# vannem95/operational-space-control

Hardware: AMD Instinct MI355X
Metric: OSC control steps/sec (batched envs), Go2 18-DoF, at 1/2/4/8 MI355X (higher is better)
Workload: dtype f64; 1 GPU; unitree_go2 standing mask=ones, 4096 envs per GPU (BASELINE configs[1]); robot=unitree_go2, envs_per_gpu=4096, global_envs=4096, parallelism=env-shard x1

## Files before the change

### operational-space-control_amd/csrc/osc_setup.hpp

```cpp
#pragma once
#include "osc_device.hpp"
#include "osc_kin_device.hpp"
#include "osc_wave_sum.hpp"

namespace osc {

typedef double d4 __attribute__((ext_vector_type(4)));

__device__ __forceinline__ double wave_sum(double v) { return wave_sum_fast(v); }

template <int NR, int NDOT>
__device__ __forceinline__ void wave_mgs(double* rows, int stride, int ncol, int lane,
                                         double drop) {
  double a[NR];
  const bool cv = lane < ncol;
#pragma unroll
  for (int w = 0; w < NR; ++w) a[w] = cv ? rows[w * stride + lane] : 0.0;
  const bool dv = lane < NDOT;
#pragma unroll
  for (int w = 0; w < NR; ++w) {
    const double n0 = sqrt(wave_sum(dv ? a[w] * a[w] : 0.0));
#pragma unroll
    for (int v = 0; v < w; ++v) {
      const double cf = wave_sum(dv ? a[v] * a[w] : 0.0);
      a[w] = fma(-cf, a[v], a[w]);
    }
    const double nn = sqrt(wave_sum(dv ? a[w] * a[w] : 0.0));
    const double sc = (nn > drop * n0 && nn > 0.0) ? 1.0 / nn : 0.0;
    a[w] *= sc;
  }
  if (cv) {
#pragma unroll
    for (int w = 0; w < NR; ++w) rows[w * stride + lane] = a[w];
  }
}

template <int NROWS, int STRIDE, int NCOL, int NDOT>
__device__ __noinline__ void wave_mgs_lds(double* rows, int lane, double drop, double* scf) {
  const bool cv = lane < NCOL, dv = lane < NDOT;
  for (int w = 0; w < NROWS; ++w) {
    double aw = cv ? rows[w * STRIDE + lane] : 0.0;
    const double n0 = sqrt(wave_sum(dv ? aw * aw : 0.0));
    for (int pass = 0; pass < 2 && w > 0; ++pass) {
      double cf = 0.0;
      if (lane < w) {
        const double* rl = rows + lane * STRIDE;
        const double* rw = rows + w * STRIDE;
#pragma unroll
        for (int c = 0; c < NDOT; ++c) cf = fma(rl[c], rw[c], cf);
      }
      if (lane < w) scf[lane] = cf;
      __builtin_amdgcn_wave_barrier();
      asm volatile("" ::: "memory");
      if (cv) {
#pragma unroll 8
        for (int v = 0; v < w; ++v) aw = fma(-scf[v], rows[v * STRIDE + lane], aw);
        rows[w * STRIDE + lane] = aw;
      }
      __builtin_amdgcn_wave_barrier();
      asm volatile("" ::: "memory");
    }
    const double nn = sqrt(wave_sum(dv ? aw * aw : 0.0));
    const double sc = (nn > drop * n0 && nn > 0.0) ? 1.0 / nn : 0.0;
    if (cv) rows[w * STRIDE + lane] = aw * sc;
    __builtin_amdgcn_wave_barrier();
    asm volatile("" ::: "memory");
  }
}

template <class D, bool KIN = false, bool LEAN = false>
__device__ __forceinline__ void setup_env(
    const DevParams* __restrict__ P, int env, int nenv, const double* __restrict__ gM,
    const double* __restrict__ gC, const double* __restrict__ gJ, const double* __restrict__ gb,
    const double* __restrict__ gT, const double* __restrict__ gmask, double* __restrict__ ws,
    double* __restrict__ sm, const double* __restrict__ gwd,
    const osc_kin::KinDev* __restrict__ Kg = nullptr, const double* __restrict__ gqpos = nullptr,
    const double* __restrict__ gqvel = nullptr) {
  constexpr int NV = D::NV, NU = D::NU, NC = D::NC, NS = D::NS, NB = D::NB, NY = D::NY,
                NY1 = D::NY1, NY1P = D::NY1P, S = D::S, NA = D::NA;
  const int lane = threadIdx.x;
  if (env >= nenv) return;

  constexpr int NAP = D::NAP;
  double* sA = sm + D::O_A;
  double* sM = sm + D::O_M;
  double* sC = sm + D::O_C;
  constexpr bool kHaG = LEAN && !D::WH && !KIN;
  double* sHa = sm + (kHaG ? D::O_HD_L : D::O_HA);
  double* sX = sm + (kHaG ? D::O_X_L : D::O_X);
  double* sU = sX + NB * NY1P;
  double* sMask = sm + (kHaG ? D::O_MASK_L : D::O_MASK);

  STAMP_DECL
  STAMP_BEGIN();
  static_assert(NV % 2 == 0 && NC % 2 == 0, "16-byte staging needs even nv and nc");
  constexpr int JC0 = 3 * (NS - NC);
  constexpr int JR0 = D::JG ? JC0 : 0;
  constexpr int KSJ = D::JG ? (S + 3) / 4 : 0;
  double jf[KSJ > 0 ? KSJ : 1];
  Batch2<NC / 2, kWave> bK;
  bK.load(gmask + static_cast<size_t>(env) * NC, lane);
  if constexpr (!KIN) {
    Batch2<D::JROWS * NV / 2, kWave> bJ;
    Batch2<NV * NV / 2, kWave> bM;
    Batch2<NV / 2, kWave> bC;
    bJ.load(gJ + static_cast<size_t>(env) * S * NV + JR0 * NV, lane);
    bM.load(gM + static_cast<size_t>(env) * NV * NV, lane);
    bC.load(gC + static_cast<size_t>(env) * NV, lane);
    {
      const int lc = lane & 15, lg = lane >> 4;
#pragma unroll
      for (int q = 0; q < KSJ; ++q) {
        const int r = 4 * q + lg;
        jf[q] = gJ[static_cast<size_t>(env) * S * NV + (r < S ? r : S - 1) * NV + (lc < NV ? lc : 0)];
      }
    }
    constexpr int TEJ = D::JG ? (S + kWave - 1) / kWave : 0;
    double ebj[TEJ > 0 ? TEJ : 1], etj[TEJ > 0 ? TEJ : 1], wj[TEJ > 0 ? TEJ : 1];
#pragma unroll
    for (int q = 0; q < TEJ; ++q) {
      const int r = (lane + q * kWave < S) ? lane + q * kWave : S - 1;
      const int half = r / (3 * NS), rr = r % (3 * NS);
      ebj[q] = gb[static_cast<size_t>(env) * S + r];
      etj[q] = gT[static_cast<size_t>(env) * NS * 6 + (rr / 3) * 6 + half * 3 + rr % 3];
      wj[q] = P->w_row[r];
    }
    constexpr int TE = D::JG ? 0 : (S + kWave - 1) / kWave;
    double eb[TE > 0 ? TE : 1], et[TE > 0 ? TE : 1];
#pragma unroll
    for (int q = 0; q < TE; ++q) {
      const int r = (lane + q * kWave < S) ? lane + q * kWave : S - 1;
      const int half = r / (3 * NS), rr = r % (3 * NS);
      eb[q] = gb[static_cast<size_t>(env) * S + r];
      et[q] = gT[static_cast<size_t>(env) * NS * 6 + (rr / 3) * 6 + half * 3 + rr % 3];
    }
    bJ.store(sA, lane, [](int c) { return (c / (NV / 2)) * (NAP / 2) + c % (NV / 2); });
#pragma unroll
    for (int q = 0; q < TEJ; ++q) {
      const int r = (lane + q * kWave < S) ? lane + q * kWave : S - 1;
      sA[D::O_E + r] = ebj[q] - etj[q];
      sA[D::O_W + r] = wj[q];
    }
    bM.store(sM, lane);
    bC.store(sC, lane);
    bK.store(sMask, lane);
    if constexpr (D::WH) {
      double* wr = ws + static_cast<size_t>(env) * D::WS;
      bM.store(wr + D::W_RM, lane);
      bC.store(wr + D::W_RC, lane);
      bJ.store(wr + D::W_RJ, lane);
      static_assert(D::JG && D::JROWS == 3 * NC, "wheel rows: the contact rows are the staged ones");
      for (int q = lane; q < 3 * NC; q += kWave) wr[D::W_RB + q] = gb[static_cast<size_t>(env) * S + JC0 + q];
      for (int q = lane; q < 6 * NC; q += kWave) wr[D::W_RD + q] = gwd[static_cast<size_t>(env) * NC * 6 + q];
    }
#pragma unroll
    for (int q = 0; q < TE; ++q) {
      const int r = (lane + q * kWave < S) ? lane + q * kWave : S - 1;
      sA[r * NAP + NV] = eb[q] - et[q];
      if (NAP > NA) sA[r * NAP + NA] = 0.0;
    }
    wave_sync();
  } else {
    osc_kin::KinDev* sK = reinterpret_cast<osc_kin::KinDev*>(sm + D::O_HA);
    {
      static_assert(sizeof(osc_kin::KinDev) % 16 == 0 && D::O_HA % 2 == 0, "16-byte staging");
      const uint4* src = reinterpret_cast<const uint4*>(Kg);
      uint4* dst = reinterpret_cast<uint4*>(sK);
      for (int i = lane; i < static_cast<int>(sizeof(osc_kin::KinDev) / 16); i += kWave)
        dst[i] = src[i];
    }
    wave_sync();
    const osc_kin::KinDev* K = sK;
    const int nq = K->nq;
    const osc_kin::EnvLayout lay(nq, NV, K->nbody, NS);
    double* E = sm + D::O_HA + sizeof(osc_kin::KinDev) / 8;
    for (int i = lane; i < nq; i += kWave) E[lay.q + i] = gqpos[static_cast<size_t>(env) * nq + i];
    for (int i = lane; i < NV; i += kWave) E[lay.q + nq + i] = gqvel[static_cast<size_t>(env) * NV + i];
    wave_sync();
    osc_kin::kin_forward(K, E, lay, lane);
    osc_kin::kin_backward(K, E, lay, lane);
    for (int d = lane; d < NV; d += kWave) sC[d] = osc_kin::kin_dof(K, E, lay, d);
    double* wr = ws + static_cast<size_t>(env) * D::WS;
    for (int k = lane; k < NS; k += kWave) {
      double bp[3], br[3];
      osc_kin::kin_site(K, E, lay, k, bp, br);
      const double* Tk = gT + static_cast<size_t>(env) * NS * 6 + k * 6;
#pragma unroll
      for (int i = 0; i < 3; ++i) {
        const int rp = 3 * k + i, rr = 3 * NS + 3 * k + i;
        if constexpr (D::JG) {
          sA[D::O_E + rp] = bp[i] - Tk[i];
          sA[D::O_E + rr] = br[i] - Tk[3 + i];
        } else {
          sA[rp * NAP + NV] = bp[i] - Tk[i];
          sA[rr * NAP + NV] = br[i] - Tk[3 + i];
          if (NAP > NA) {
            sA[rp * NAP + NA] = 0.0;
            sA[rr * NAP + NA] = 0.0;
          }
        }
        if constexpr (D::WH) {
          if (k >= NS - NC) wr[D::W_RB + 3 * (k - (NS - NC)) + i] = bp[i];
        }
      }
    }
    if constexpr (D::JG) {
      for (int r = lane; r < S; r += kWave) sA[D::O_W + r] = P->w_row[r];
    }
    wave_sync();
    {
      const int j = lane & 31, par = lane >> 5;
      const bool vj = j < NV;
      const double* Dj = E + lay.dof + osc_kin::kDofStride * (vj ? j : 0);
      double Sj[6], Fj[6];
#pragma unroll
      for (int t = 0; t < 6; ++t) {
        Sj[t] = Dj[t];
        Fj[t] = Dj[6 + t];
      }
      for (int i = par; i < NV; i += 2) {
        const double* Di = E + lay.dof + osc_kin::kDofStride * i;
        double Si[6], Fi[6];
#pragma unroll
        for (int t = 0; t < 6; ++t) {
          Si[t] = Di[t];
          Fi[t] = Di[6 + t];
        }
        const double m = osc_kin::kin_m_entry(K->dof_relmask[i], K->dof_arm[i], i, j, Si, Fi, Sj, Fj);
        if (vj) sM[i * NV + j] = m;
      }
      for (int k = (D::JG ? NS - NC : 0) + par; k < NS; k += 2) {
        const double* xs = E + lay.site + 3 * k;
        const double xk[3] = {xs[0], xs[1], xs[2]};
        double jp[3], jr[3];
        osc_kin::kin_j_col(vj && ((K->site_dofmask[k] >> j) & 1u), Sj, xk, jp, jr);
        if (vj) {
#pragma unroll
          for (int t = 0; t < 3; ++t) {
            sA[(3 * k + t - JR0) * NAP + j] = jp[t];
            if (!D::JG) sA[(3 * NS + 3 * k + t) * NAP + j] = jr[t];
          }
        }
      }
      if constexpr (D::JG) {
        const int lc = lane & 15, lg = lane >> 4;
        const int c = lc < NV ? lc : 0;
        const double* Dc = E + lay.dof + osc_kin::kDofStride * c;
        double Sc[6];
#pragma unroll
        for (int t = 0; t < 6; ++t) Sc[t] = Dc[t];
#pragma unroll
        for (int q = 0; q < KSJ; ++q) {
          const int r0 = 4 * q + lg, r = r0 < S ? r0 : S - 1;
          const int half = r / (3 * NS), rr = r % (3 * NS), k = rr / 3, t = rr % 3;
          const double* xs = E + lay.site + 3 * k;
          const double xk[3] = {xs[0], xs[1], xs[2]};
          double jp[3], jr[3];
          osc_kin::kin_j_col((K->site_dofmask[k] >> c) & 1u, Sc, xk, jp, jr);
          jf[q] = half ? jr[t] : jp[t];
        }
      }
    }
    wave_sync();
    bK.store(sMask, lane);
    wave_sync();
    if constexpr (D::WH) {
      for (int q = lane; q < NV * NV; q += kWave) wr[D::W_RM + q] = sM[q];
      for (int q = lane; q < NV; q += kWave) wr[D::W_RC + q] = sC[q];
      for (int q = lane; q < 3 * NC * NV; q += kWave)
        wr[D::W_RJ + q] = sA[(q / NV) * NAP + q % NV];
      for (int q = lane; q < 6 * NC; q += kWave) wr[D::W_RD + q] = gwd[static_cast<size_t>(env) * NC * 6 + q];
    }
  }

  STAMP_END(0);
  STAMP_BEGIN();
  double* const wha = ws + static_cast<size_t>(env) * D::WS;
  auto put_ha = [&](int i, int j, double v) {
    if (i >= NA || j >= NA) return;
    v *= 2.0;
    if (i == j && i < NV) v += 2.0 * P->w_reg;
    if constexpr (kHaG) {
      if (j < NV) {
        sHa[i * NV + j] = v;
        sHa[j * NV + i] = v;
      }
    } else {
      sHa[i * NA + j] = v;
      sHa[j * NA + i] = v;
    }
    if (j < NV) {
      wha[D::W_HD + i * NV + j] = v;
      wha[D::W_HD + j * NV + i] = v;
    } else if (j == NV && i < NV) {
      wha[D::W_GD + i] = v;
    }
  };
  if constexpr (D::JG) {
    constexpr int NBK = (NA + 15) / 16, KS = (S + 3) / 4;
    const int lc = lane & 15, lg = lane >> 4;
    d4 acc[NBK * (NBK + 1) / 2];
#pragma unroll
    for (int t = 0; t < NBK * (NBK + 1) / 2; ++t) acc[t] = d4{0.0, 0.0, 0.0, 0.0};
    constexpr int CH = 8;
#pragma unroll
    for (int q0 = 0; q0 < KS; q0 += CH) {
      double v[CH][NBK], wv[CH];
#pragma unroll
      for (int u = 0; u < CH; ++u) {
        const int r = 4 * (q0 + u) + lg;
        const bool rv = r < S;
        wv[u] = rv ? sA[D::O_W + r] : 0.0;
#pragma unroll
        for (int b = 0; b < NBK; ++b) {
          const int col = 16 * b + lc;
          const double ev = sA[D::O_E + (rv ? r : 0)];
          v[u][b] = !rv ? 0.0 : (col < NV ? jf[q0 + u < KSJ ? q0 + u : 0] : (col == NV ? ev : 0.0));
        }
      }
#pragma unroll
      for (int u = 0; u < CH; ++u) {
        if (q0 + u >= KS) break;
        int t = 0;
#pragma unroll
        for (int bi = 0; bi < NBK; ++bi)
#pragma unroll
          for (int bj = bi; bj < NBK; ++bj, ++t)
            acc[t] = __builtin_amdgcn_mfma_f64_16x16x4f64(wv[u] * v[u][bi], v[u][bj], acc[t], 0, 0, 0);
      }
    }
    int t = 0;
#pragma unroll
    for (int bi = 0; bi < NBK; ++bi)
#pragma unroll
      for (int bj = bi; bj < NBK; ++bj, ++t)
#pragma unroll
        for (int rr = 0; rr < 4; ++rr) {
          const int i = 16 * bi + lg + 4 * rr, j = 16 * bj + lc;
          if (i <= j) put_ha(i, j, acc[t][rr]);
        }
  } else
  for (int p = lane; p < D::NBA; p += kWave) {
    int i0, j0;
    upper_pair<D::NA2>(p, i0, j0);
    i0 *= 2;
    j0 *= 2;
    double a00 = 0.0, a01 = 0.0, a10 = 0.0, a11 = 0.0;
    auto ha_row = [&](int r) {
      const double2 x = *reinterpret_cast<const double2*>(sA + r * NAP + i0);
      const double2 y = *reinterpret_cast<const double2*>(sA + r * NAP + j0);
      const double w = P->w_row[r];
      const double wx0 = w * x.x, wx1 = w * x.y;
      a00 = fma(wx0, y.x, a00);
      a01 = fma(wx0, y.y, a01);
      a10 = fma(wx1, y.x, a10);
      a11 = fma(wx1, y.y, a11);
    };
    if constexpr (LEAN) {
#pragma unroll 4
      for (int r = 0; r < S; ++r) ha_row(r);
    } else {
      for (int r = 0; r < S; ++r) ha_row(r);
    }
    put_ha(i0, j0, a00);
    put_ha(i0, j0 + 1, a01);
    if (i0 != j0) put_ha(i0 + 1, j0, a10);
    put_ha(i0 + 1, j0 + 1, a11);
  }

  STAMP_END(1);
  STAMP_BEGIN();
  constexpr bool kSplitU = 2 * NY1P <= kWave;
  constexpr int kUStep = kSplitU ? (NU + 1) / 2 : NU;
  const int c = kSplitU ? (lane & 31) : lane;
  const int a_lo = kSplitU ? (lane >> 5) * kUStep : 0;
  double x[NB];
  double uacc[kUStep];
#pragma unroll
  for (int i = 0; i < NB; ++i) x[i] = 0.0;
#pragma unroll
  for (int t = 0; t < kUStep; ++t) uacc[t] = 0.0;
  if (c < NY1) {
    const bool pinned = (c >= NU && c < NY) && (sMask[(c - NU) / 3] == 0.0);
    const bool cu = c < NU, cz = !cu && c < NY;
    const double* xp = cu ? sM + NB + c : (cz ? sA + (JC0 - JR0 + c - NU) * NAP : sC);
    const int xs = cu ? NV : 1;
    const double xsg = cz ? 1.0 : -1.0;
    const double* up =
        cu ? sM + NB * NV + NB + c : (cz ? sA + (JC0 - JR0 + c - NU) * NAP + NB : sC + NB);
    const double usg = cz ? -1.0 : 1.0;
#pragma unroll
    for (int i = 0; i < NB; ++i) x[i] = pinned ? 0.0 : xsg * xp[i * xs];
    double L[NB][NB];
    double dinv[NB];
#pragma unroll
    for (int i = 0; i < NB; ++i)
#pragma unroll
      for (int j = 0; j <= i; ++j) L[i][j] = sM[i * NV + j];
#pragma unroll
    for (int k = 0; k < NB; ++k) {
      dinv[k] = L[k][k] > 0.0 ? recip1(L[k][k]) : __builtin_nan("");
#pragma unroll
      for (int i = k + 1; i < NB; ++i) {
        const double lik = L[i][k] * dinv[k];
#pragma unroll
        for (int j = k + 1; j <= i; ++j) L[i][j] = fma(-lik, L[j][k], L[i][j]);
      }
#pragma unroll
      for (int i = k + 1; i < NB; ++i) L[i][k] *= dinv[k];
    }
#pragma unroll
    for (int k = 0; k < NB; ++k)
#pragma unroll
      for (int i = k + 1; i < NB; ++i) x[i] = fma(-L[i][k], x[k], x[i]);
#pragma unroll
    for (int k = 0; k < NB; ++k) x[k] *= dinv[k];
#pragma unroll
    for (int k = NB - 1; k >= 0; --k)
#pragma unroll
      for (int i = 0; i < k; ++i) x[i] = fma(-L[k][i], x[k], x[i]);
    if (!kHaG && a_lo == 0) {
#pragma unroll
      for (int i = 0; i < NB; ++i) sX[i * NY1P + c] = x[i];
    }
#pragma unroll
    for (int t = 0; t < kUStep; ++t) {
      const int a = a_lo + t;
      if (a < NU) {
        double acc = pinned ? 0.0 : usg * up[a * xs];
#pragma unroll
        for (int i = 0; i < NB; ++i) acc = fma(sM[(NB + a) * NV + i], x[i], acc);
        if constexpr (kHaG) uacc[t] = acc;
        else sU[a * NY1P + c] = acc;
      }
    }
  }
  if constexpr (kHaG) wave_sync();
  if (kHaG ? c < NY1P : (c >= NY1 && c < NY1P)) {
    if (a_lo == 0) {
#pragma unroll
      for (int i = 0; i < NB; ++i) sX[i * NY1P + c] = x[i];
    }
#pragma unroll
    for (int t = 0; t < kUStep; ++t)
      if (a_lo + t < NU) sU[(a_lo + t) * NY1P + c] = uacc[t];
  }
  wave_sync();
  {
    static_assert(NU <= kRow, "S fits one 16-lane row");
    STAMP_END(2);
    STAMP_BEGIN();
    const int lj = lane & (kRow - 1);
    double col[NU];
#pragma unroll
    for (int i = 0; i < NU; ++i) col[i] = sU[i * NY1P + (lj < NU ? lj : 0)];
    double dj = 1.0;
    static_for<0, NU>([&](auto K) {
      constexpr int k = decltype(K)::value;
      const double pk = bcast_guarded<k>(col[k]);
      const double rk = pk > 0.0 ? recip1(pk) : __builtin_nan("");
      if (lj == k) dj = rk;
      const double m = (lj > k) ? -col[k] * rk : 0.0;
      static_for<k + 1, NU>([&](auto I) {
        constexpr int i = decltype(I)::value;
        fmac_bcast_self<k, true>(col[i], m);
      });
    });
    double dinv[NU];
    static_for<0, NU>([&](auto K) {
      constexpr int k = decltype(K)::value;
      dinv[k] = bcast_guarded<k>(dj);
    });
    STAMP_END(6);
    STAMP_BEGIN();
    const int c = lane;
    const bool cu = c < NU, live = c < NY1;
    const int cc = (cu || !live) ? NU : c;
    double xa[NU], xb[NB], xbc[NB];
#pragma unroll
    for (int i = 0; i < NU; ++i) {
      const double u = sU[i * NY1P + cc];
      xa[i] = cu ? ((i == c) ? 1.0 : 0.0) : -u;
    }
#pragma unroll
    for (int r = 0; r < NB; ++r) {
      xb[r] = sX[r * NY1P + cc];
      xbc[r] = sX[r * NY1P + (lj < NU ? lj : 0)];
    }
    static_for<0, NU>([&](auto K) {
      constexpr int k = decltype(K)::value;
      const double t = -xa[k] * dinv[k];
      static_for<k + 1, NU>([&](auto I) {
        constexpr int i = decltype(I)::value;
        fmac_bcast<k>(xa[i], col[i], t);
      });
    });
#pragma unroll
    for (int k = 0; k < NU; ++k) xa[k] *= dinv[k];
    static_for<0, NU - 1>([&](auto J) {
      constexpr int i = NU - 2 - decltype(J)::value;
      double acc = 0.0;
      static_for<i + 1, NU>([&](auto K) {
        constexpr int k = decltype(K)::value;
        fmac_bcast<i>(acc, col[k], xa[k]);
      });
      xa[i] = fma(-dinv[i], acc, xa[i]);
    });
    STAMP_END(7);
    STAMP_BEGIN();
#pragma unroll
    for (int r = 0; r < NB; ++r) xb[r] = cu ? 0.0 : xb[r];
    static_for<0, NU>([&](auto Q) {
      constexpr int q = decltype(Q)::value;
#pragma unroll
      for (int r = 0; r < NB; ++r) fmac_bcast<q>(xb[r], xbc[r], xa[q]);
    });
    wave_sync();
    if (c < NY1P) {
      double* const wx = ws + static_cast<size_t>(env) * D::WS + D::W_X;
#pragma unroll
      for (int r = 0; r < NB; ++r) {
        const double v = live ? xb[r] : 0.0;
        sX[r * NY1P + c] = v;
        wx[r * NY1P + c] = v;
      }
#pragma unroll
      for (int i = 0; i < NU; ++i) {
        const double v = live ? xa[i] : 0.0;
        sX[(NB + i) * NY1P + c] = v;
        wx[(NB + i) * NY1P + c] = v;
      }
    }
    wave_sync();
    STAMP_END(8);
    STAMP_BEGIN();
  }
  if constexpr (D::WH) {
    static_assert(D::JG && D::NW <= kRow, "wheel rows: contact rows of J staged in LDS");
    constexpr int NW = D::NW, WEST = D::WEST, WAST = D::WAST;
    double* sWE = sm + D::O_WE;
    double* sWA = sm + D::O_WA;
    const double* wd = gwd + static_cast<size_t>(env) * NC * 6;
    for (int p = lane; p < NW * WEST; p += kWave) {
      const int w = p / WEST, c = p % WEST;
      const int i = w >> 1, side = w & 1;
      double acc = 0.0;
      if (c <= NV) {
#pragma unroll
        for (int q = 0; q < 3; ++q) {
          const double dc = wd[i * 6 + side * 3 + q];
          const double v = (c == NV) ? gb[static_cast<size_t>(env) * S + JC0 + 3 * i + q]
                                     : sA[(3 * i + q) * NAP + c];
          acc = fma(dc, v, acc);
        }
        if (c < NV && side == 0 && c == P->wheel_dof[i]) acc -= P->wheel_radius[i];
        acc *= (c == NV) ? -sMask[i] : sMask[i];
      } else {
        acc = (c - NV - 1 == w) ? 1.0 : 0.0;
      }
      sWE[p] = acc;
    }
    wave_sync();
    wave_mgs<NW, NV>(sWE, WEST, NV + 1 + NW, lane, 1e-9);
    wave_sync();
    int rank = 0;
#pragma unroll
    for (int w = 0; w < NW; ++w) rank += (sWE[w * WEST + w + NV + 1] != 0.0) ? 1 : 0;
    for (int p = lane; p < NW * WAST; p += kWave) {
      const int w = p / WAST, c = p % WAST;
      double acc;
      if (c < NY1P) {
        acc = (c == NY) ? -sWE[w * WEST + NV] : 0.0;
#pragma unroll
        for (int j = 0; j < NV; ++j) acc = fma(sWE[w * WEST + j], sX[j * NY1P + c], acc);
      } else {
        acc = (c - NY1P == w) ? 1.0 : 0.0;
      }
      sWA[p] = acc;
    }
    wave_sync();
    double* const wx = ws + static_cast<size_t>(env) * D::WS + D::W_X;
    for (int p = lane; p < NV * NY1P; p += kWave) {
      const int j = p / NY1P, c = p % NY1P;
      double v = sX[p];
#pragma unroll
      for (int w = 0; w < NW; ++w) v = fma(-sWE[w * WEST + j], sWA[w * WAST + c], v);
      v = (rank == NV && c < NY) ? 0.0 : v;
      sX[p] = v;
      wx[p] = v;
    }
    wave_sync();
    wave_mgs<NW, NY>(sWA, WAST, WAST, lane, 1e-9);
    wave_sync();
    double* const wsw = ws + static_cast<size_t>(env) * D::WS;
    for (int p = lane; p < NW * NY1P; p += kWave)
      wsw[D::W_AW + p] = sWA[(p / NY1P) * WAST + p % NY1P];
    for (int p = lane; p < NW * NV; p += kWave) wsw[D::W_WV + p] = sWE[(p / NV) * WEST + p % NV];
    for (int p = lane; p < NW * NW; p += kWave) {
      const int w = p / NW, c = p % NW;
      wsw[D::W_WR + p] = sWE[w * WEST + NV + 1 + c];
      wsw[D::W_WL + p] = sWA[w * WAST + NY1P + c];
    }
    STAMP_END(9);
    STAMP_BEGIN();
    constexpr int TS = D::WTST;
    double* sWT = sm + D::O_WT;
    for (int p = lane; p < (NW + NY) * NY; p += kWave) {
      const int w = p / NY, c = p % NY;
      sWT[w * TS + c] = (w < NW) ? sWA[w * WAST + c] : ((c == w - NW) ? 1.0 : 0.0);
    }
    wave_sync();
    wave_mgs_lds<NW + NY, TS, NY, NY>(sWT, lane, 1e-9, sWE);
    wave_sync();
    int kept = 0;
    for (int w = 0; w < NW + NY; ++w) {
      const double a = lane < NY ? sWT[w * TS + lane] : 0.0;
      if (wave_sum(a * a) > 0.0) {
        if (kept < NY) {
          if (lane < NY) sWT[kept * TS + lane] = a;
          if (lane == 0) wsw[D::W_PIN + kept] = (w < NW) ? static_cast<double>(w) : -1.0;
        }
        ++kept;
      }
      wave_sync();
    }
    for (int k = kept; k < NY; ++k) {
      if (lane < NY) sWT[k * TS + lane] = 0.0;
      if (lane == 0) wsw[D::W_PIN + k] = -2.0;
    }
    wave_sync();
    for (int p = lane; p < NY * NY; p += kWave) {
      const int i = p / NY, k = p % NY;
      wsw[D::W_T + p] = sWT[k * TS + i];
    }
    STAMP_END(10);
    STAMP_BEGIN();
    for (int p = lane; p < NV * NY; p += kWave) {
      const int j = p / NY, k = p % NY;
      double v = 0.0;
#pragma unroll 8
      for (int i = 0; i < NY; ++i) v = fma(sX[j * NY1P + i], sWT[k * TS + i], v);
      sWE[p] = v;
    }
    wave_sync();
    for (int p = lane; p < NV * NY; p += kWave) {
      const int j = p / NY, k = p % NY;
      sX[j * NY1P + k] = sWE[p];
      wx[j * NY1P + k] = sWE[p];
    }
    wave_sync();
  }

  STAMP_END(2);
  STAMP_BEGIN();
  if constexpr (kHaG) __builtin_amdgcn_fence(__ATOMIC_SEQ_CST, "workgroup");
  {
    constexpr int RB = (NV + 15) / 16, CB = (NY1P + 15) / 16, KS = (NV + 3) / 4;
    const int lc = lane & 15, lg = lane >> 4;
    double xf[KS][CB];
    double hf[RB][KS];
#pragma unroll
    for (int q = 0; q < KS; ++q) {
      const int k = 4 * q + lg;
      const bool kv = k < NV;
#pragma unroll
      for (int cb = 0; cb < CB; ++cb) {
        const int col = 16 * cb + lc;
        const double x = sX[(kv ? k : 0) * NY1P + (col < NY1P ? col : 0)];
        xf[q][cb] = (kv && col < NY1P) ? x : 0.0;
      }
#pragma unroll
      for (int rb = 0; rb < RB; ++rb) {
        const int row = 16 * rb + lc;
        const int hr = row < NV ? row : 0, hk = kv ? k : 0;
        const double h = sHa[hr * (kHaG ? NV : NA) + hk];
        hf[rb][q] = (kv && row < NV) ? h : 0.0;
      }
    }
    d4 t1[RB][CB];
#pragma unroll
    for (int rb = 0; rb < RB; ++rb)
#pragma unroll
      for (int cb = 0; cb < CB; ++cb)
#pragma unroll
        for (int rr = 0; rr < 4; ++rr) {
          const int row = 16 * rb + lg + 4 * rr, col = 16 * cb + lc;
          const double f = kHaG ? wha[D::W_GD + (row < NV ? row : 0)]
                                : sHa[(row < NV ? row : 0) * NA + NV];
          t1[rb][cb][rr] = (row < NV && col == NY) ? f : 0.0;
        }
#pragma unroll
    for (int q = 0; q < KS; ++q)
#pragma unroll
      for (int rb = 0; rb < RB; ++rb)
#pragma unroll
        for (int cb = 0; cb < CB; ++cb)
          t1[rb][cb] = __builtin_amdgcn_mfma_f64_16x16x4f64(hf[rb][q], xf[q][cb], t1[rb][cb], 0, 0, 0);
    const double wu2 = 2.0 * (P->w_torque + P->w_reg);
    const double wr2 = 2.0 * P->w_reg;
    double* wsv = ws + static_cast<size_t>(env) * D::WS;
    auto store_hr = [&](int a, int b, double v) {
      if constexpr (!D::HRC) {
        wsv[D::W_HR + a * NY + b] = v;
        wsv[D::W_HR + b * NY + a] = v;
      } else if (b >= kRow) {
        wsv[D::W_HR + hr_off<D>(b, a)] = v;
        if (a >= kRow && a != b) wsv[D::W_HR + hr_off<D>(a, b)] = v;
      } else {
        wsv[D::W_HR + hr_off<D>(a, b)] = v;
      }
    };
    constexpr int NT = CB * (CB + 1) / 2;
    d4 hacc[NT];
#pragma unroll
    for (int t = 0; t < NT; ++t) hacc[t] = d4{0.0, 0.0, 0.0, 0.0};
#pragma unroll
    for (int q = 0; q < KS; ++q) {
      int t = 0;
#pragma unroll
      for (int ab = 0; ab < CB; ++ab)
#pragma unroll
        for (int bb = ab; bb < CB; ++bb, ++t)
          hacc[t] = __builtin_amdgcn_mfma_f64_16x16x4f64(xf[q][ab], t1[q / 4][bb][q % 4], hacc[t],
                                                         0, 0, 0);
    }
    int tt = 0;
#pragma unroll
    for (int ab = 0; ab < CB; ++ab)
#pragma unroll
      for (int bb = ab; bb < CB; ++bb, ++tt) {
        const d4 h = hacc[tt];
#pragma unroll
        for (int rr = 0; rr < 4; ++rr) {
          const int a = 16 * ab + lg + 4 * rr, b = 16 * bb + lc;
          const int kz = (a >= NU) ? (a - NU) / 3 : 0;
          const double mk = sMask[kz < NC ? kz : NC - 1];
          double v = h[rr];
          if (a <= b && b < NY1 && !(a == NY && b == NY)) {
            if (b < NY && D::WH) {
              const double* sT = sm + D::O_WT;
              double wab = 0.0;
#pragma unroll 8
              for (int i = 0; i < NY; ++i) {
                const int ki = (i >= NU) ? (i - NU) / 3 : 0;
                const double wi = (i < NU) ? wu2 : (sMask[ki] == 0.0 ? 1.0 : wr2);
                wab = fma(wi * sT[a * D::WTST + i], sT[b * D::WTST + i], wab);
              }
              v += wab;
              store_hr(a, b, v);
            } else if (b < NY) {
              if (a == b && a < NU) v += wu2;
              if (a == b && a >= NU) v = (mk == 0.0) ? 1.0 : v + wr2;
              store_hr(a, b, v);
            } else {
              wsv[D::W_G + a] = v;
            }
          }
        }
      }
    wave_sync();
  }

  STAMP_END(4);
  STAMP_BEGIN();
  STAMP_END(5);
  STAMP_STORE_SETUP();
}

#ifndef OSC_SETUP_WPS
#define OSC_SETUP_WPS 2
#endif
#ifndef OSC_SETUP_LEAN_WPS
#define OSC_SETUP_LEAN_WPS 4
#endif
template <class D, bool LEAN = false>
__global__ __launch_bounds__(kWave, LEAN ? OSC_SETUP_LEAN_WPS : OSC_SETUP_WPS) void osc_setup_kernel(
    const DevParams* __restrict__ P, int nenv, const double* __restrict__ gM,
    const double* __restrict__ gC, const double* __restrict__ gJ, const double* __restrict__ gb,
    const double* __restrict__ gT, const double* __restrict__ gmask, double* __restrict__ ws,
    const double* __restrict__ gwd) {
  __shared__ __attribute__((aligned(16))) double sm[(LEAN && !D::WH) ? D::SMEM_L : D::SMEM];
  setup_env<D, false, LEAN>(P, static_cast<int>(blockIdx.x), nenv, gM, gC, gJ, gb, gT, gmask, ws,
                            sm, gwd);
}

extern __shared__ __attribute__((aligned(16))) double osc_setup_qpos_sm[];
template <class D>
__global__ __launch_bounds__(kWave, 2) void osc_setup_qpos_kernel(
    const DevParams* __restrict__ P, int nenv, const osc_kin::KinDev* __restrict__ Kg,
    const double* __restrict__ gqpos, const double* __restrict__ gqvel,
    const double* __restrict__ gT, const double* __restrict__ gmask, double* __restrict__ ws,
    const double* __restrict__ gwd) {
  setup_env<D, true>(P, static_cast<int>(blockIdx.x), nenv, nullptr, nullptr, nullptr, nullptr, gT,
                     gmask, ws, osc_setup_qpos_sm, gwd, Kg, gqpos, gqvel);
}
template <class D>
inline int kin_lds_doubles(int nq, int nbody) {
  const int kin = D::O_HA + static_cast<int>(sizeof(osc_kin::KinDev) / 8) +
                  osc_kin::EnvLayout(nq, D::NV, nbody, D::NS).size;
  return kin > D::SMEM ? kin : D::SMEM;
}

template <class DA, class DB>
__global__ __launch_bounds__(kWave, 2) void osc_setup_pair_kernel(PairArgs A, PairArgs B) {
  __shared__ __attribute__((aligned(16))) double sm[cmax(DA::SMEM, DB::SMEM)];
  const int blk = static_cast<int>(blockIdx.x);
  if (blk < A.nenv)
    setup_env<DA>(A.P, blk, A.nenv, A.M, A.C, A.J, A.b, A.T, A.mask, A.ws, sm, nullptr);
  else
    setup_env<DB>(B.P, blk - A.nenv, B.nenv, B.M, B.C, B.J, B.b, B.T, B.mask, B.ws, sm, nullptr);
}

}
```

Baseline: 31.06 million solves/s.

## Software-pipeline Hessian accumulation and hoist loads ahead of dependent math in setup

Replaces the per-row Hessian-block accumulation loop in the lean non-JG path with a double-buffered, five-row software pipeline. Row weights are held one per lane and broadcast with readlane instead of being reloaded from parameters. Shared-memory loads of x/u vectors and mask values are hoisted ahead of the factorization and MFMA epilogue, and diagonal-regularization branches are turned into selects, with values pinned in VGPRs. The aim is to hide LDS latency and cut divergent branches, at the cost of more registers, possibly lower occupancy, and a constraint that S be a multiple of ten.

```diff
diff --git a/operational-space-control_amd/csrc/osc_setup.hpp b/operational-space-control_amd/csrc/osc_setup.hpp
--- a/operational-space-control_amd/csrc/osc_setup.hpp
+++ b/operational-space-control_amd/csrc/osc_setup.hpp
@@ -66,6 +66,15 @@
     __builtin_amdgcn_wave_barrier();
     asm volatile("" ::: "memory");
   }
+}
+
+template <int N>
+__device__ __forceinline__ void upper_pair_int(int p, int& i, int& j) {
+  int r = 0;
+#pragma unroll
+  for (int k = 1; k < N; ++k) r += (p >= k * (2 * N - k + 1) / 2) ? 1 : 0;
+  i = r;
+  j = p - r * (2 * N - r + 1) / 2 + r;
 }
 
 template <class D, bool KIN = false, bool LEAN = false>
@@ -100,6 +109,11 @@
   double jf[KSJ > 0 ? KSJ : 1];
   Batch2<NC / 2, kWave> bK;
   bK.load(gmask + static_cast<size_t>(env) * NC, lane);
+  const double wreg2 = 2.0 * P->w_reg;
+  constexpr bool kBPipe = LEAN && !D::JG && !KIN;
+  static_assert(!kBPipe || S <= kWave, "one row weight per lane");
+  double wl = 0.0;
+  if constexpr (kBPipe) wl = P->w_row[lane < S ? lane : S - 1];
   if constexpr (!KIN) {
     Batch2<D::JROWS * NV / 2, kWave> bJ;
     Batch2<NV * NV / 2, kWave> bM;
@@ -159,6 +173,7 @@
       sA[r * NAP + NV] = eb[q] - et[q];
       if (NAP > NA) sA[r * NAP + NA] = 0.0;
     }
+    if constexpr (kBPipe) in_vgpr(wl);
     wave_sync();
   } else {
     osc_kin::KinDev* sK = reinterpret_cast<osc_kin::KinDev*>(sm + D::O_HA);
@@ -279,21 +294,28 @@
   auto put_ha = [&](int i, int j, double v) {
     if (i >= NA || j >= NA) return;
     v *= 2.0;
-    if (i == j && i < NV) v += 2.0 * P->w_reg;
     if constexpr (kHaG) {
+      double vd = v + wreg2;
+      in_vgpr(vd);
+      v = (i == j && i < NV) ? vd : v;
       if (j < NV) {
         sHa[i * NV + j] = v;
         sHa[j * NV + i] = v;
+        wha[D::W_HD + i * NV + j] = v;
+        wha[D::W_HD + j * NV + i] = v;
+      } else if (i < NV) {
+        wha[D::W_GD + i] = v;
       }
     } else {
+      if (i == j && i < NV) v += wreg2;
       sHa[i * NA + j] = v;
       sHa[j * NA + i] = v;
-    }
-    if (j < NV) {
-      wha[D::W_HD + i * NV + j] = v;
-      wha[D::W_HD + j * NV + i] = v;
-    } else if (j == NV && i < NV) {
-      wha[D::W_GD + i] = v;
+      if (j < NV) {
+        wha[D::W_HD + i * NV + j] = v;
+        wha[D::W_HD + j * NV + i] = v;
+      } else if (j == NV && i < NV) {
+        wha[D::W_GD + i] = v;
+      }
     }
   };
   if constexpr (D::JG) {
@@ -342,25 +364,46 @@
   } else
   for (int p = lane; p < D::NBA; p += kWave) {
     int i0, j0;
-    upper_pair<D::NA2>(p, i0, j0);
+    upper_pair_int<D::NA2>(p, i0, j0);
     i0 *= 2;
     j0 *= 2;
     double a00 = 0.0, a01 = 0.0, a10 = 0.0, a11 = 0.0;
-    auto ha_row = [&](int r) {
-      const double2 x = *reinterpret_cast<const double2*>(sA + r * NAP + i0);
-      const double2 y = *reinterpret_cast<const double2*>(sA + r * NAP + j0);
-      const double w = P->w_row[r];
+    auto ha_mac = [&](double2 x, double2 y, double w) {
       const double wx0 = w * x.x, wx1 = w * x.y;
       a00 = fma(wx0, y.x, a00);
       a01 = fma(wx0, y.y, a01);
       a10 = fma(wx1, y.x, a10);
       a11 = fma(wx1, y.y, a11);
     };
-    if constexpr (LEAN) {
-#pragma unroll 4
-      for (int r = 0; r < S; ++r) ha_row(r);
+    if constexpr (kBPipe) {
+      constexpr int kBU = 5;
+      static_assert(S % (2 * kBU) == 0, "phase B: whole double stages");
+      const double* const px = sA + i0;
+      const double* const py = sA + j0;
+      double2 xs0[kBU], ys0[kBU], xs1[kBU], ys1[kBU];
+      auto ld = [&](double2 (&xv)[kBU], double2 (&yv)[kBU], int r0) {
+#pragma unroll
+        for (int u = 0; u < kBU; ++u) {
+          xv[u] = *reinterpret_cast<const double2*>(px + (r0 + u) * NAP);
+          yv[u] = *reinterpret_cast<const double2*>(py + (r0 + u) * NAP);
+        }
+      };
+      auto mac = [&](const double2 (&xv)[kBU], const double2 (&yv)[kBU], int r0) {
+#pragma unroll
+        for (int u = 0; u < kBU; ++u) ha_mac(xv[u], yv[u], readlane_d(wl, r0 + u));
+      };
+      ld(xs0, ys0, 0);
+#pragma unroll 1
+      for (int r0 = 0; r0 < S; r0 += 2 * kBU) {
+        ld(xs1, ys1, r0 + kBU);
+        mac(xs0, ys0, r0);
+        ld(xs0, ys0, r0 + 2 * kBU < S ? r0 + 2 * kBU : 0);
+        mac(xs1, ys1, r0 + kBU);
+      }
     } else {
-      for (int r = 0; r < S; ++r) ha_row(r);
+      for (int r = 0; r < S; ++r)
+        ha_mac(*reinterpret_cast<const double2*>(sA + r * NAP + i0),
+               *reinterpret_cast<const double2*>(sA + r * NAP + j0), P->w_row[r]);
     }
     put_ha(i0, j0, a00);
     put_ha(i0, j0 + 1, a01);
@@ -389,8 +432,11 @@
     const double* up =
         cu ? sM + NB * NV + NB + c : (cz ? sA + (JC0 - JR0 + c - NU) * NAP + NB : sC + NB);
     const double usg = cz ? -1.0 : 1.0;
-#pragma unroll
-    for (int i = 0; i < NB; ++i) x[i] = pinned ? 0.0 : xsg * xp[i * xs];
+    double xr[NB], u0[kUStep];
+#pragma unroll
+    for (int i = 0; i < NB; ++i) xr[i] = xp[i * xs];
+#pragma unroll
+    for (int t = 0; t < kUStep; ++t) u0[t] = up[(a_lo + t < NU ? a_lo + t : NU - 1) * xs];
     double L[NB][NB];
     double dinv[NB];
 #pragma unroll
@@ -398,6 +444,13 @@
 #pragma unroll
       for (int j = 0; j <= i; ++j) L[i][j] = sM[i * NV + j];
 #pragma unroll
+    for (int i = 0; i < NB; ++i) {
+      in_vgpr(xr[i]);
+      x[i] = pinned ? 0.0 : xsg * xr[i];
+    }
+#pragma unroll
+    for (int t = 0; t < kUStep; ++t) in_vgpr(u0[t]);
+#pragma unroll
     for (int k = 0; k < NB; ++k) {
       dinv[k] = L[k][k] > 0.0 ? recip1(L[k][k]) : __builtin_nan("");
 #pragma unroll
@@ -426,12 +479,14 @@
 #pragma unroll
     for (int t = 0; t < kUStep; ++t) {
       const int a = a_lo + t;
-      if (a < NU) {
-        double acc = pinned ? 0.0 : usg * up[a * xs];
-#pragma unroll
-        for (int i = 0; i < NB; ++i) acc = fma(sM[(NB + a) * NV + i], x[i], acc);
-        if constexpr (kHaG) uacc[t] = acc;
-        else sU[a * NY1P + c] = acc;
+      const double* const mrow = sM + (NB + (a < NU ? a : NU - 1)) * NV;
+      double acc = pinned ? 0.0 : usg * u0[t];
+#pragma unroll
+      for (int i = 0; i < NB; ++i) acc = fma(mrow[i], x[i], acc);
+      if constexpr (kHaG) {
+        uacc[t] = acc;
+      } else {
+        if (a < NU) sU[a * NY1P + c] = acc;
       }
     }
   }
@@ -478,15 +533,19 @@
     const int cc = (cu || !live) ? NU : c;
     double xa[NU], xb[NB], xbc[NB];
 #pragma unroll
-    for (int i = 0; i < NU; ++i) {
-      const double u = sU[i * NY1P + cc];
-      xa[i] = cu ? ((i == c) ? 1.0 : 0.0) : -u;
-    }
+    for (int i = 0; i < NU; ++i) xa[i] = sU[i * NY1P + cc];
 #pragma unroll
     for (int r = 0; r < NB; ++r) {
       xb[r] = sX[r * NY1P + cc];
       xbc[r] = sX[r * NY1P + (lj < NU ? lj : 0)];
     }
+#pragma unroll
+    for (int i = 0; i < NU; ++i) {
+      in_vgpr(xa[i]);
+      xa[i] = cu ? ((i == c) ? 1.0 : 0.0) : -xa[i];
+    }
+#pragma unroll
+    for (int r = 0; r < NB; ++r) in_vgpr(xb[r]);
     static_for<0, NU>([&](auto K) {
       constexpr int k = decltype(K)::value;
       const double t = -xa[k] * dinv[k];
@@ -697,7 +756,7 @@
         for (int cb = 0; cb < CB; ++cb)
           t1[rb][cb] = __builtin_amdgcn_mfma_f64_16x16x4f64(hf[rb][q], xf[q][cb], t1[rb][cb], 0, 0, 0);
     const double wu2 = 2.0 * (P->w_torque + P->w_reg);
-    const double wr2 = 2.0 * P->w_reg;
+    const double wr2 = wreg2;
     double* wsv = ws + static_cast<size_t>(env) * D::WS;
     auto store_hr = [&](int a, int b, double v) {
       if constexpr (!D::HRC) {
@@ -711,6 +770,15 @@
       }
     };
     constexpr int NT = CB * (CB + 1) / 2;
+    double mkv[CB][4];
+#pragma unroll
+    for (int ab = 0; ab < CB; ++ab)
+#pragma unroll
+      for (int rr = 0; rr < 4; ++rr) {
+        const int a = 16 * ab + lg + 4 * rr;
+        const int kz = (a >= NU) ? (a - NU) / 3 : 0;
+        mkv[ab][rr] = sMask[kz < NC ? kz : NC - 1];
+      }
     d4 hacc[NT];
 #pragma unroll
     for (int t = 0; t < NT; ++t) hacc[t] = d4{0.0, 0.0, 0.0, 0.0};
@@ -733,8 +801,7 @@
 #pragma unroll
         for (int rr = 0; rr < 4; ++rr) {
           const int a = 16 * ab + lg + 4 * rr, b = 16 * bb + lc;
-          const int kz = (a >= NU) ? (a - NU) / 3 : 0;
-          const double mk = sMask[kz < NC ? kz : NC - 1];
+          const double mk = mkv[ab][rr];
           double v = h[rr];
           if (a <= b && b < NY1 && !(a == NY && b == NY)) {
             if (b < NY && D::WH) {
@@ -749,8 +816,11 @@
               v += wab;
               store_hr(a, b, v);
             } else if (b < NY) {
-              if (a == b && a < NU) v += wu2;
-              if (a == b && a >= NU) v = (mk == 0.0) ? 1.0 : v + wr2;
+              double vu = v + wu2, vz = v + wr2;
+              in_vgpr(vu);
+              in_vgpr(vz);
+              vz = (mk == 0.0) ? 1.0 : vz;
+              v = (a == b) ? (a < NU ? vu : vz) : v;
               store_hr(a, b, v);
             } else {
               wsv[D::W_G + a] = v;
```

Result: no change. 31.31 million solves/s, median of 6 (+0.8%).
